# ethereum/pos-evolution

Hardware: AMD Instinct MI355X
Metric: attestations aggregated/sec + get_head() p50 latency at 1M validators (higher is better)
Workload: dtype int32

## Files before the change

pos_evolution_amd/csrc/engine_g1.cpp:

```cpp
#include "engine_internal.h"

using namespace posevo;

namespace posevo {

void g1_stream_guard(pe_engine* h, hipStream_t s)
{
    if (h->side_ever && s != h->side_stream && s != h->fin_stream && s != h->norm_stream) (void)hipStreamWaitEvent(s, h->ev_join, 0);
}

int build_points30(pe_engine* h, uint64_t n)
{
    HIP_TRY(h, h->d_points30.ensure(std::max<size_t>(128, 4ull * G1_ROW_WORDS * n)));
    launch_g1_table_s30(h->stream, h->d_points.as<uint32_t>(), h->d_points30.as<uint32_t>(), n);
    HIP_TRY(h, hipGetLastError());
    h->points30_valid = true;
    return PE_OK;
}

int launch_g1_planned(pe_engine* h, const uint32_t* d_points, const uint32_t* d_members, const uint32_t* d_bits,
                      const G1Group* d_groups, const G1Plan& plan, uint8_t* d_out96, uint32_t* dev_jac,
                      hipStream_t s, hipStream_t fin, DevBuf* partials, DevBuf* lane_partials, const AttPlan* plan_dev,
                      const uint32_t* d_members1, uint64_t caller_rows, const G1Complement* cm)
{
    if (plan.n_groups == 0) return PE_OK;
    if (!s) s = h->stream;
    if (!fin) fin = s;
    if (!partials) partials = &h->d_partials;
    if (!lane_partials) lane_partials = &h->d_lane_partials;
    PE_TRY(ensure_quiesced(h, *partials,
                           std::max<size_t>(PE_G1_PARTIAL_BYTES, (size_t)PE_G1_PARTIAL_BYTES * plan.n_partials)));
    const size_t lane_bytes = (size_t)G1_LANE_PARTIAL_BYTES * G1_WG * ((plan.n_slots + G1_WG - 1) / G1_WG);
    PE_TRY(ensure_quiesced(h, *lane_partials, std::max<size_t>(PE_G1_PARTIAL_BYTES, lane_bytes)));
    const uint32_t* d_points30;
    if (d_points == h->d_points.as<uint32_t>()) {
        if (!h->points30_valid) return fail(h, PE_ERR_STATE, "the registry's table of the accumulation's field form was not built");
        d_points30 = h->d_points30.as<uint32_t>();
    } else {
        const uint64_t n_rows = caller_rows;
        if (d_points != h->d_tmp_points.as<uint32_t>() || 4ull * G1_ROW_WORDS * n_rows > h->d_tmp_points.cap)
            return fail(h, PE_ERR_STATE, "G1 sum over an unknown point table");
        HIP_TRY(h, h->d_tmp_points30.ensure(std::max<size_t>(128, 4ull * G1_ROW_WORDS * n_rows)));
        launch_g1_table_s30(s, d_points, h->d_tmp_points30.as<uint32_t>(), n_rows);
        d_points30 = h->d_tmp_points30.as<uint32_t>();
    }
    const bool chain = fin != s && fin == h->fin_stream;
    const int exclusive = chain && h->tune.exclusive && h->blocks.size() <= 4096 ? 1 : 0;
    {
        const bool skip = !h->prof_timeline && s != h->stream && (h->acc_launches++ & 3) != 0;
        ProfScope ps(h, PE_KERNEL_G1_ACCUMULATE, s, skip);
        unsigned long long* clock_rec = nullptr;
        if (h->profiling) {
            if (!h->acc_clock && hipHostMalloc(reinterpret_cast<void**>(&h->acc_clock), 16ull * pe_engine::ACC_CLOCK_RING,
                                               hipHostMallocDefault) != hipSuccess) {
                (void)hipGetLastError();
                h->acc_clock = nullptr;
            }
            if (h->acc_clock) {
                clock_rec = h->acc_clock + 2 * (h->acc_clock_n++ % pe_engine::ACC_CLOCK_RING);
                clock_rec[0] = clock_rec[1] = 0;
            }
        }
        launch_g1_accumulate(s, d_points30, d_members, d_bits, d_groups, plan.n_groups, plan.n_slots,
                             lane_partials->as<uint32_t>(), partials->as<uint32_t>(), plan_dev, d_members1, exclusive, clock_rec,
                             cm ? cm->cmpl : nullptr);
    }
    hipStream_t ts = fin;
    if (ts != s) {
        HIP_TRY(h, hipEventRecord(h->ev_acc, s));
        HIP_TRY(h, hipStreamWaitEvent(ts, h->ev_acc, 0));
    }
    {
        ProfScope ps(h, PE_KERNEL_G1_TREE, ts);
        launch_g1_tree(ts, lane_partials->as<uint32_t>(), d_groups, plan.n_groups, plan.n_slots, partials->as<uint32_t>(),
                       ts != s ? 1 : 0,
                       plan_dev, exclusive);
    }
    hipStream_t ns = fin;
    if (chain && h->norm_stream) {
        ns = h->norm_stream;
        HIP_TRY(h, hipEventRecord(h->ev_tree, ts));
        HIP_TRY(h, hipStreamWaitEvent(ns, h->ev_tree, 0));
    } else if (ts != fin) {
        HIP_TRY(h, hipEventRecord(h->ev_tree, ts));
        HIP_TRY(h, hipStreamWaitEvent(fin, h->ev_tree, 0));
    }
    if (cm)
        for (int t = 0; t < 2; ++t)
            if (cm->ev[t]) HIP_TRY(h, hipStreamWaitEvent(ns, cm->ev[t], 0));
    {
        ProfScope ps(h, PE_KERNEL_G1_NORMALISE, ns);
        launch_g1_finish(ns, partials->as<uint32_t>(), d_groups, plan.n_groups, 0, 0, d_out96, dev_jac, plan_dev,
                         cm ? cm->cmpl : nullptr, cm ? cm->sums[0] : nullptr, cm ? cm->sums[1] : nullptr);
    }
    HIP_TRY(h, hipGetLastError());
    return PE_OK;
}

void committee_sums_drop(pe_engine* h)
{
    for (auto& t : h->tables) t.sums_valid = t.sums_wanted = false;
    if (h->sums_stream) (void)hipStreamSynchronize(h->sums_stream);
}
int build_committee_sums(pe_engine* h, CommitteeTable* t, bool defer)
{
    t->sums_valid = false;
    t->sums_wanted = false;
    if (!h->tune.committee_sums || !t->is_partition || !h->have_points || !h->points30_valid || h->dist_ready()) return PE_OK;
    if (t->n_committees == 0 || t->n_val_at_load != h->n_val || t->offsets.size() != (size_t)t->n_committees + 1) return PE_OK;
// ... 681 lines not shown
```

pos_evolution_amd/csrc/engine_internal.h:

```cpp
#pragma once
#include <hip/hip_runtime.h>
#include <dlfcn.h>
#include <rccl/rccl.h>

#include <algorithm>
#include <array>
#include <chrono>
#include <cstdlib>
#include <map>
#include <cstdio>
#include <cstddef>
#include <cstring>
#include <functional>
#include <memory>
#include <new>
#include <numeric>
#include <string>
#include <thread>
#include <unordered_map>
#include <vector>

#include "../../include/posevo.h"
#include "../../include/posevo_profile.h"
#include "att_row.h"
// ... 330 lines not shown
    };
    std::vector<SigSeg> sig_batch;
    hipEvent_t ev_sig = nullptr;
    hipEvent_t ev_fork = nullptr, ev_join = nullptr;
    bool side_busy = false;
    bool side_ever = false;
    bool streaming = false;
    std::vector<std::function<int()>> deferred;
    struct HeldFc {
        bool active = false;
        int arena = -1;
        bool have_fc = false;
        bool have_head = false;
        ValidateFcArgs validate{};
        LmdVmArgs lmd{};
        VotesArgs votes{};
        TreeArgs tree{};
        std::function<int()> between;
        std::vector<std::function<int()>> g1;
        bool fence_pending = false;
    } held;
    bool pairing = std::getenv("POSEVO_PAIR") == nullptr || std::atoi(std::getenv("POSEVO_PAIR")) != 0;
    struct Tune {
        static int env(const char* name, int dflt)
        {
            const char* e = std::getenv(name);
            return e && *e ? std::atoi(e) : dflt;
        }
        int exclusive = env("POSEVO_ACC_EXCLUSIVE", 1);
        int state_on = env("POSEVO_STATE_ON", 2);
        int sig_batch = env("POSEVO_SIG_BATCH", 8);
        int queue_probe = env("POSEVO_QUEUE_PROBE", 1);
        int committee_sums = env("POSEVO_COMMITTEE_SUMS", 1);
        uint32_t ssz_tile_log2 = (uint32_t)std::min<int>(SSZ_TILE_LOG2, std::max<int>(SSZ_TILE_LOG2_MIN, env("POSEVO_SSZ_TILE_LOG2", SSZ_TILE_LOG2)));
    } tune;

    struct ResGroup { uint32_t byte_off, n_bits, word, sig_valid, tag; };
    std::vector<ResGroup> res_groups;
    std::shared_ptr<std::vector<uint32_t>> res_info_host;
    bool res_valid = false;
    int res_arena = 0;
    uint64_t res_generation = 0;

    struct ResidentRows {
        bool valid = false;
        int arena = 0;
        uint32_t n_in = 0;
        const void* rows = nullptr;
        TablesDev tables{};
        uint64_t generation = 0;
        int set = 0;
        uint32_t n_groups = 0;
    } rr;

    int g1_tune_calls = 0;
    float g1_tune_best[2] = {1e30f, 1e30f};
    uint32_t g1_target_slots = 0;
    hipEvent_t g1_tune_ev[2] = {nullptr, nullptr};
    bool points30_valid = false;
    DevBuf d_points30, d_tmp_points30;

    ncclComm_t comm = nullptr, comm_g1 = nullptr;
    int early_rc = PE_OK;
    uint32_t xchg_blocks = 0;
    uint64_t xchg_nval = 0;
    bool last_agg_on_side = false;
// ... 300 lines not shown
            d.slot_base = cursor;
            d.out_base = outp;
            continue;
        }
        if (d.n_tasks <= wg_slots) {
            uint32_t l2 = 0;
            while ((1u << l2) < d.n_tasks) ++l2;
            d.log2_block = l2;
            const uint32_t blk = 1u << l2;
            cursor = (cursor + blk - 1) & ~(blk - 1);
            d.slot_base = cursor;
            cursor += blk;
            d.out_base = outp;
            outp += 1;
        } else {
            d.log2_block = 9;
            cursor = (cursor + wg_slots - 1) & ~(wg_slots - 1);
            d.slot_base = cursor;
            const uint32_t wgs = (d.n_tasks + wg_slots - 1) / wg_slots;
            cursor += wgs * wg_slots;
            d.out_base = outp;
            outp += wgs;
        }
    }
    plan->n_groups = n_groups;
    plan->n_slots = cursor;
    plan->n_partials = outp;
}

void g1_stream_guard(pe_engine* h, hipStream_t s);
int build_points30(pe_engine* h, uint64_t n);
struct G1Complement {
    const uint32_t* cmpl = nullptr;
    const uint32_t* sums[2] = {nullptr, nullptr};
    hipEvent_t ev[2] = {nullptr, nullptr};
};
int launch_g1_planned(pe_engine* h, const uint32_t* d_points, const uint32_t* d_members, const uint32_t* d_bits,
                      const G1Group* d_groups, const G1Plan& plan, uint8_t* d_out96, uint32_t* dev_jac,
                      hipStream_t s = nullptr, hipStream_t fin = nullptr, DevBuf* partials = nullptr,
                      DevBuf* lane_partials = nullptr, const AttPlan* plan_dev = nullptr,
                      const uint32_t* d_members1 = nullptr, uint64_t caller_rows = 0, const G1Complement* cm = nullptr);
int build_committee_sums(pe_engine* h, CommitteeTable* t, bool defer);
int committee_sums_build_wanted(pe_engine* h, CommitteeTable* t);
void committee_sums_drop(pe_engine* h);

struct Resolved {
    CommitteeTable* table = nullptr;
    uint32_t pos = 0;
    uint32_t size = 0;
    uint32_t block_idx = 0;
};
inline CommitteePos resolve_committee(const pe_engine* h, CommitteeTable* t, const pe_attestation& a, Resolved* out)
{
    const CommitteePos cp = att_committee_pos(t->n_committees, h->cfg.slots_per_epoch, a.slot, a.index);
    if (cp.exists) {
        out->table = t;
        out->pos = cp.pos;
        out->size = t->offsets[cp.pos + 1] - t->offsets[cp.pos];
    }
    return cp;
}

struct BatchMemo {
    struct Slot { uint8_t root[32]; uint32_t idx; uint32_t used; };
    Slot slots[256];
    std::vector<uint64_t> anc;
// ... 91 lines not shown
```

pos_evolution_amd/csrc/engine_resident.cpp:

```cpp
#include "engine_internal.h"


using namespace posevo;

namespace posevo {

namespace {

struct RrLayout {
    AttPlan* plan;
    uint32_t *slot_of, *rep_of, *gid_of_row, *ubytes, *member_row;
    PlanSync* sync;
    PlanRec* rec;
    AttGroup* grp;
    UnionGroup* ug;
    G1Group* g1;
    AttRow *rows_fc, *rows_st;
    int32_t *status_fc, *status_st;
    uint32_t* cmpl;
    uint32_t *crow_start[2], *crow_cursor[2], *crow_cnt[2], *crow_list[2];
    size_t bytes;
};

RrLayout rr_layout(uint8_t* base, uint32_t cap_n, uint32_t cap_c)
// ... 181 lines not shown
    const uint32_t slot_cap = std::max<uint32_t>(2 * G1_TARGET_LANES, (n + G1_WG - 1) / G1_WG * G1_WG);
    const size_t words_cap = (size_t)out_arena_cap / 4 + n + 16;
    Stage st(h);
    PE_TRY(st.reserve((size_t)arena_len + 256));
    const size_t pad_at = ((size_t)arena_len + 15) & ~size_t(15);
    const size_t off_arena = st.alloc(pad_at + 32);
    if (set == 0) {
        PE_TRY(ensure_quiesced_arenas(h, &pe_engine::PipeArena::d_res_bits, words_cap * 4 + 64));
        PE_TRY(ensure_quiesced_arenas(h, &pe_engine::PipeArena::d_res_info, 8ull * n + 64));
    } else {
        PE_TRY(ensure_quiesced(h, RS.bits, words_cap * 4 + 64));
        PE_TRY(ensure_quiesced(h, RS.info, 8ull * n + 64));
    }
    OutBlock ob(h);
    const size_t off_plan = ob.alloc(sizeof(AttPlan));
    const size_t off_rows = ob.alloc(sizeof(pe_attestation) * (size_t)n);
    const size_t off_gof = ob.alloc(4ull * n);
    const size_t off_obits = ob.alloc(words_cap * 4);
    const size_t off_oinfo = ob.alloc(8ull * n);
    const size_t off_opk = out_aggpk96 ? ob.alloc(96ull * n) : 0;
    G1Complement cm;
    bool by_cmpl = false;
    if (out_aggpk96 && !dev_partials && set == 0 && h->tune.committee_sums && !h->dist_ready())
        for (int t = 0; t < 2; ++t) {
            if (tabs[t]) PE_TRY(committee_sums_build_wanted(h, tabs[t]));
            if (tabs[t] && tabs[t]->sums_valid && tabs[t]->d_sums.p && tabs[t]->ev_sums) {
                cm.sums[t] = tabs[t]->d_sums.as<uint32_t>();
                cm.ev[t] = tabs[t]->ev_sums;
                by_cmpl = true;
            }
        }
    const size_t off_ocm = by_cmpl ? ob.alloc(4ull * n) : 0;
    PE_TRY(ob.ensure());
    if (by_cmpl) cm.cmpl = L.cmpl;
    if (want_pk) {
        PE_TRY(ensure_quiesced_arenas(h, &pe_engine::PipeArena::d_partials, std::max<size_t>(PE_G1_PARTIAL_BYTES, (size_t)PE_G1_PARTIAL_BYTES * n)));
        PE_TRY(ensure_quiesced_arenas(h, &pe_engine::PipeArena::d_lane_partials, (size_t)G1_LANE_PARTIAL_BYTES * slot_cap));
        PE_TRY(ensure_quiesced(h, h->d_partials, std::max<size_t>(PE_G1_PARTIAL_BYTES, (size_t)PE_G1_PARTIAL_BYTES * n)));
        PE_TRY(ensure_quiesced(h, h->d_lane_partials, (size_t)G1_LANE_PARTIAL_BYTES * slot_cap));
    }
    lap.mark("ragg.1_reserve");
    *out_n_groups = 0;
    AttPlan* plan_host = ob.host<AttPlan>(off_plan);
    memset(plan_host, 0, sizeof(AttPlan));
    plan_host->error = 0xFFFFFFFFu;
    const MemKind arena_kind = arena_len ? mem_kind(bits_arena) : MemKind::Pageable;
    hipStream_t ms = h->stream;
    const bool pair_ok = h->held.active && h->held.arena != h->cur && set == 0 && !n_dev && hold_eligible(h);
    if (h->held.active && !pair_ok) PE_TRY(held_issue(h));
    if (set == 0) {
        if (!h->deferred.empty()) PE_TRY(run_deferred(h));
        if (A.side_used) HIP_TRY(h, hipStreamWaitEvent(ms, h->ev_join, 0));
        if (sig_batch_holds(h, h->cur)) PE_TRY(sig_batch_flush(h));
        if (A.leg_used) HIP_TRY(h, hipStreamWaitEvent(ms, A.ev_leg, 0));
        PE_TRY(aux_join(h, ms));
    }
    h->res_valid = false;
    h->rr.valid = false;
    const size_t deferred_before = h->deferred.size();
    struct Unwind {
        pe_engine* h; size_t keep; bool armed = true;
        ~Unwind() { if (armed) { h->rr.valid = false; if (h->deferred.size() > keep) h->deferred.resize(keep); } }
    } unwind{h, deferred_before};
    bool ingest_copies = false;
    if (arena_kind == MemKind::Pageable) {
        memcpy(st.host<uint8_t>(off_arena), bits_arena, arena_len);
        memset(st.host<uint8_t>(off_arena) + arena_len, 0, pad_at + 32 - arena_len);
// ... 328 lines not shown
```

pos_evolution_amd/csrc/g1_kernels.hip:

```cpp
#define POSEVO_FP_MUL_CALLED 1
#include <algorithm>
#include <hip/hip_ext.h>
#include "g1.h"
#include "g1_s30.h"
#include "fp_sqrt.h"
#include "kernels.h"

namespace posevo {

__global__ void __launch_bounds__(256) k_g1_convert(const uint8_t* __restrict__ be96, uint32_t* __restrict__ mont24,
                                                     uint64_t n)
{
    uint64_t i = (uint64_t)blockIdx.x * blockDim.x + threadIdx.x;
    if (i >= n) return;
    const uint8_t* src = be96 + 96 * i;
    uint32_t* dst = mont24 + (uint64_t)G1_ROW_WORDS * i;
    if (src[0] & 0x40) {
#pragma unroll
        for (int j = 0; j < 24; ++j) dst[j] = 0;
        return;
    }
    fp x, y, xm, ym;
    fp_load_be48(x, src);
    fp_load_be48(y, src + 48);
    y.l[11] = __builtin_bswap32(reinterpret_cast<const uint32_t*>(src + 48)[0]);
    fp_to_mont(xm, x);
    fp_to_mont(ym, y);
#pragma unroll
    for (int j = 0; j < 12; ++j) {
        dst[j] = xm.l[j];
        dst[12 + j] = ym.l[j];
    }
}

void launch_g1_convert(hipStream_t s, const uint8_t* be96, uint32_t* mont24, uint64_t n)
{
    if (n == 0) return;
    hipLaunchKernelGGL(k_g1_convert, dim3((unsigned)((n + 255) / 256)), dim3(256), 0, s, be96, mont24, n);
}
// ... 162 lines not shown
__device__ __forceinline__ void global_store_x(uint32_t* __restrict__ dst, const g1x& p)
{
    global_store_fp(dst, p.x);
    global_store_fp(dst + 12, p.y);
    global_store_fp(dst + 24, p.zz);
    global_store_fp(dst + 36, p.zzz);
}
__device__ __forceinline__ void global_load_x(g1x& p, const uint32_t* __restrict__ src)
{
    global_load_fp(p.x, src);
    global_load_fp(p.y, src + 12);
    global_load_fp(p.zz, src + 24);
    global_load_fp(p.zzz, src + 36);
}

__device__ __forceinline__ uint32_t find_group(const G1Group* __restrict__ groups, uint32_t n_groups, uint32_t slot)
{
    uint32_t lo = 0, hi = n_groups;
    {
        const uint32_t lb = groups[0].log2_block;
        const uint32_t g0 = min(lb <= 8 ? slot >> lb : 0u, n_groups - 1);
        if (groups[g0].slot_base <= slot) {
            if (g0 + 1 == n_groups || groups[g0 + 1].slot_base > slot) return g0;
            lo = g0 + 1;
        } else {
            hi = g0;
        }
    }
    while (hi - lo > 1) {
        uint32_t mid = (lo + hi) >> 1;
        if (groups[mid].slot_base <= slot) lo = mid; else hi = mid;
    }
    return lo;
}

#ifdef POSEVO_G1_PHASE_TIMING
__device__ unsigned long long g1_phase_stamps[16 * 4096];
#define G1_STAMP(i) do { if (threadIdx.x == 0 && blockIdx.x < 4096) g1_phase_stamps[blockIdx.x * 16 + (i)] = wall_clock64(); } while (0)
__device__ unsigned long long g1_wave_info[3 * 4 * 4096];
#define G1_WAVE_BEGIN() do { if ((threadIdx.x & 63) == 0 && blockIdx.x < 4096) { \
        unsigned long long* w_ = &g1_wave_info[3 * (blockIdx.x * 4 + (threadIdx.x >> 6))]; \
        w_[0] = (unsigned long long)__builtin_amdgcn_s_getreg((4) | (0 << 6) | (31 << 11)) | \
                ((unsigned long long)__builtin_amdgcn_s_getreg((20) | (0 << 6) | (31 << 11)) << 32); \
        w_[1] = wall_clock64(); } } while (0)
#define G1_WAVE_END() do { if ((threadIdx.x & 63) == 0 && blockIdx.x < 4096) \
        g1_wave_info[3 * (blockIdx.x * 4 + (threadIdx.x >> 6)) + 2] = wall_clock64(); } while (0)
#else
#define G1_WAVE_BEGIN() do { } while (0)
#define G1_WAVE_END() do { } while (0)
#define G1_STAMP(i) do { } while (0)
#endif

namespace s30 {
__device__ __noinline__ fq fq_mul_nc(int32_t a0, int32_t a1, int32_t a2, int32_t a3, int32_t a4, int32_t a5, int32_t a6,
                                     int32_t a7, int32_t a8, int32_t a9, int32_t a10, int32_t a11, int32_t a12,
                                     int32_t b0, int32_t b1, int32_t b2, int32_t b3, int32_t b4, int32_t b5, int32_t b6,
                                     int32_t b7, int32_t b8, int32_t b9, int32_t b10, int32_t b11, int32_t b12)
{
    const fq a = {{a0, a1, a2, a3, a4, a5, a6, a7, a8, a9, a10, a11, a12}};
    const fq b = {{b0, b1, b2, b3, b4, b5, b6, b7, b8, b9, b10, b11, b12}};
    fq r;
    fq_mul(r, a, b);
    return r;
}
__device__ __noinline__ fq fq_sqr_nc(int32_t a0, int32_t a1, int32_t a2, int32_t a3, int32_t a4, int32_t a5, int32_t a6,
                                     int32_t a7, int32_t a8, int32_t a9, int32_t a10, int32_t a11, int32_t a12)
// ... 146 lines not shown
    fq_from_lane(t2, m4, base);
    fq_sub_norm(tmp, m4, t2);
    fq_select(sel, q == 1, m3, m4);
    fq_select(out_a, q == 2, X3, sel);
    out_b = tmp;
    return true;
}

__device__ __forceinline__ void g1_slot_block(const G1Group* __restrict__ groups, uint32_t n_groups, uint32_t n_slots,
                                              uint32_t slot, uint32_t& my_out, uint32_t& my_size, G1Group& d, uint32_t& t,
                                              uint32_t* g_out = nullptr)
{
    my_out = NONE32;
    my_size = 0;
    t = 0;
    if (slot >= n_slots) return;
    const uint32_t g = find_group(groups, n_groups, slot);
    if (g_out) *g_out = g;
    d = groups[g];
    t = slot - d.slot_base;
    const bool wide = d.log2_block > 8;
    const uint32_t block_slots = d.n_tasks == 0 ? 0u
                               : wide ? ((d.n_tasks + G1_WG - 1) / G1_WG) * G1_WG : (1u << d.log2_block);
    if (t < block_slots) {
        my_size = wide ? (uint32_t)G1_WG : (1u << d.log2_block);
        my_out = d.out_base + (wide ? (t >> 8) : 0u);
    }
}


template <bool SOLO>
__device__ __forceinline__ void g1_tree_body(const uint32_t* __restrict__ lane_partials, const G1Group* __restrict__ groups,
                                             uint32_t n_groups, uint32_t n_slots, uint32_t* __restrict__ wg_partials,
                                             const AttPlan* __restrict__ plan_dev)
{
    if (SOLO) asm volatile("" ::: "a7");
    if (plan_dev) {
        n_groups = plan_dev->n_groups;
        n_slots = plan_dev->n_slots;
    }
    extern __shared__ __attribute__((aligned(16))) uint32_t lds[];
    uint32_t* lds_out = lds + G1S_WORDS * G1_WG;
    uint32_t* lds_sz = lds_out + G1_WG;
    const int tid = threadIdx.x;
    for (uint32_t wg = blockIdx.x; wg * G1_WG < n_slots; wg += gridDim.x) {
    const uint32_t slot = wg * G1_WG + tid;
    uint32_t my_out, my_size, t;
    G1Group d{};
    g1_slot_block(groups, n_groups, n_slots, slot, my_out, my_size, d, t);
    if (my_size == 1) my_size = 0;
    {
        const uint32_t* b = lane_partials + (size_t)wg * G1S_WORDS * G1_WG + tid;
#pragma unroll
        for (int k = 0; k < G1S_WORDS; ++k) lds[k * G1_WG + tid] = b[k * G1_WG];
    }
    lds_out[tid] = my_out;
    lds_sz[tid] = my_size;
    __syncthreads();
    G1_STAMP(2);
#ifdef POSEVO_G1_PHASE_TIMING
    int g1_level = 0;
#endif
    for (int n = G1_WG / 2; n >= 1; n >>= 1) {
        if (n <= G1_WG / 4) {
            const int w = tid >> 2, q = tid & 3;
            const bool active = w < n;
            fq out_a, out_b;
            uint32_t out = NONE32, sz = 0;
            bool store_lds = false;
            if (active) {
                sz = lds_sz[2 * w];
                out = lds_out[2 * w];
                if (sz >= 2) {
                    fq a, b;
                    lds_load_fq(a, lds, q >> 1, 2 * w + (q & 1));
                    lds_load_fq(b, lds, 2 + (q >> 1), 2 * w + ((q & 1) ^ 1));
                    const unsigned long long inf_lanes = __ballot(fq_limbs_zero(b));
                    bool fast = ((inf_lanes >> ((tid & 63) & ~3)) & 0xFull) == 0;
                    if (fast) fast = g1s_add_quad(out_a, out_b, q, a, b);
                    if (!fast) {
                        g1q p1, p2;
                        lds_load_q(p1, lds, 2 * w);
                        lds_load_q(p2, lds, 2 * w + 1);
                        g1q_add_full(p1, p2);
                        if (p1.inf) g1q_set_inf(p1);
                        fq sel;
                        fq_select(sel, q == 1, p1.zz, p1.zzz);
                        fq_select(out_a, q == 2, p1.x, sel);
                        out_b = p1.y;
                    }
                    sz >>= 1;
// ... 67 lines not shown
                    global_store_fq_as_mont32(dst, out_a);
                    global_store_fq_as_mont32(dst + 12, out_b);
                    sz = 0;
                } else {
                    store_lds = true;
                }
            } else {
                sz = 0;
            }
        }
        __syncthreads();
        if (active) {
            if (store_lds) {
                lds_store_fq(lds, role ? 2 : 0, w, out_a);
                lds_store_fq(lds, role ? 3 : 1, w, out_b);
            }
            if (!role) {
                lds_out[w] = out;
                lds_sz[w] = sz;
            }
        }
        __syncthreads();
#ifdef POSEVO_G1_PHASE_TIMING
        G1_STAMP(3 + g1_level);
        ++g1_level;
#endif
    }
    }
}
}

__global__ void __launch_bounds__(G1_WG) __attribute__((amdgpu_waves_per_eu(2, 2)))
k_g1_tree(const uint32_t* __restrict__ lane_partials, const G1Group* __restrict__ groups, uint32_t n_groups,
          uint32_t n_slots, uint32_t* __restrict__ wg_partials, const AttPlan* __restrict__ plan_dev)
{
    s30::g1_tree_body<false>(lane_partials, groups, n_groups, n_slots, wg_partials, plan_dev);
}
__global__ void __launch_bounds__(G1_WG) __attribute__((amdgpu_waves_per_eu(1, 1), amdgpu_num_vgpr(256)))
k_g1_tree_solo(const uint32_t* __restrict__ lane_partials, const G1Group* __restrict__ groups, uint32_t n_groups,
               uint32_t n_slots, uint32_t* __restrict__ wg_partials, const AttPlan* __restrict__ plan_dev)
{
    s30::g1_tree_body<true>(lane_partials, groups, n_groups, n_slots, wg_partials, plan_dev);
}

__global__ void __launch_bounds__(256)
k_g1_table_s30(const uint32_t* __restrict__ pts32, uint32_t* __restrict__ pts30, uint64_t n)
{
    using s30::FQ_N;
    const uint64_t i = (uint64_t)blockIdx.x * 256 + threadIdx.x;
    if (i >= n) return;
    const uint32_t* src = pts32 + (uint64_t)G1_ROW_WORDS * i;
    uint32_t w[24], any = 0;
#pragma unroll
    for (int k = 0; k < 24; ++k) { w[k] = src[k]; any |= w[k]; }
    uint32_t* dst = pts30 + (uint64_t)G1_ROW_WORDS * i;
    s30::fq x, y;
    s30::fq_set_zero(x);
    s30::fq_set_zero(y);
    if (any) {
        s30::fq_from_mont32(x, w);
        s30::fq_from_mont32(y, w + 12);
    }
#pragma unroll
    for (int k = 0; k < FQ_N; ++k) { dst[k] = (uint32_t)x.l[k]; dst[FQ_N + k] = (uint32_t)y.l[k]; }
    dst[2 * FQ_N] = any ? 1u : 0u;
#pragma unroll
    for (int k = 2 * FQ_N + 1; k < G1_ROW_WORDS; ++k) dst[k] = 0;
}

namespace s30 {
static_assert(2 * FQ_N + 1 <= 28, "a row of the S30 table is read as seven 16-byte vectors");
__device__ __forceinline__ bool load_point_s30(fq& x, fq& y, const uint32_t* __restrict__ pts30, uint32_t idx)
{
    const uint4* p = reinterpret_cast<const uint4*>(pts30 + (uint64_t)G1_ROW_WORDS * idx);
    const uint4 v0 = p[0], v1 = p[1], v2 = p[2], v3 = p[3], v4 = p[4], v5 = p[5], v6 = p[6];
    x.l[0] = v0.x; x.l[1] = v0.y; x.l[2] = v0.z; x.l[3] = v0.w;
    x.l[4] = v1.x; x.l[5] = v1.y; x.l[6] = v1.z; x.l[7] = v1.w;
    x.l[8] = v2.x; x.l[9] = v2.y; x.l[10] = v2.z; x.l[11] = v2.w;
    x.l[12] = v3.x;
    y.l[0] = v3.y; y.l[1] = v3.z; y.l[2] = v3.w;
    y.l[3] = v4.x; y.l[4] = v4.y; y.l[5] = v4.z; y.l[6] = v4.w;
    y.l[7] = v5.x; y.l[8] = v5.y; y.l[9] = v5.z; y.l[10] = v5.w;
    y.l[11] = v6.x; y.l[12] = v6.y;
    return v6.z != 0;
}
}

namespace s30 {
__device__ __forceinline__ void g1_accumulate_body(const uint32_t* __restrict__ pts30, const uint32_t* __restrict__ members,
                                                   const uint32_t* __restrict__ bit_arena, const G1Group* __restrict__ groups,
                                                   uint32_t n_groups, uint32_t n_slots, uint32_t* __restrict__ lane_partials,
                                                   uint32_t* __restrict__ wg_partials, const AttPlan* __restrict__ plan_dev,
                                                   const uint32_t* __restrict__ members1,
                                                   unsigned long long* __restrict__ clock_rec,
                                                   const uint32_t* __restrict__ cmpl)
{
    const int tid = threadIdx.x;
    if (plan_dev) {
        n_groups = plan_dev->n_groups;
        n_slots = plan_dev->n_slots;
        if (blockIdx.x * G1_WG >= n_slots) return;
    }
    unsigned long long rec_w0 = 0, rec_c0 = 0;
    if (clock_rec && blockIdx.x == 0) {
        rec_w0 = wall_clock64();
        rec_c0 = clock64();
    }
    const uint32_t slot = blockIdx.x * G1_WG + tid;
    G1_STAMP(0);
    G1_WAVE_BEGIN();
#ifdef POSEVO_ACC_PRIO_LEVEL
    __builtin_amdgcn_s_setprio(POSEVO_ACC_PRIO_LEVEL);
#endif
    g1q acc;
    g1q_set_inf(acc);
    bool exc = false;
    uint32_t my_out, my_size, t;
    G1Group d{};
    uint32_t g = 0;
    g1_slot_block(groups, n_groups, n_slots, slot, my_out, my_size, d, t, &g);
    uint32_t first = 0, count = 0;
    uint32_t invert = 0;
    if (slot < n_slots && t < d.n_tasks) {
        const uint32_t gk = d.k & 0x7FFFFFFFu;
        if (d.k >> 31) members = members1;
        first = t * gk;
        count = min(gk, d.n_members - first);
        if (cmpl) invert = cmpl[g] != NONE32 ? 1u : 0u;
    }
    const bool gated = d.bits_word != NONE32;
    auto want = [&](uint32_t j, uint32_t& idx) -> bool {
        const uint32_t i = first + j;
        idx = members ? members[d.member_start + i] : d.member_start + i;
        if (!gated) return true;
        return (((bit_arena[d.bits_word + (i >> 5)] >> (i & 31)) & 1u) ^ invert) != 0;
    };
    auto fetch = [&](uint32_t j, fq& ox, fq& oy) -> bool {
        uint32_t idx;
        if (!want(j, idx)) return false;
        return load_point_s30(ox, oy, pts30, idx);
    };
    {
        fq qx, qy, nx, ny;
        bool have = false, nhave = false, w1 = false, w2 = false;
        uint32_t i1 = 0, i2 = 0;
        if (count > 0) {
            uint32_t i0;
            if (want(0, i0)) have = load_point_s30(qx, qy, pts30, i0);
        }
        if (count > 1) w1 = want(1, i1);
        for (uint32_t j = 0; j < count; ++j) {
            w2 = false;
            if (j + 2 < count) w2 = want(j + 2, i2);
            nhave = false;
            if (w1) nhave = load_point_s30(nx, ny, pts30, i1);
            if (have) {
                if (acc.inf) g1q_set_first(acc, qx, qy);
                else g1q_madd_fast(acc, qx, qy, exc);
            }
            qx = nx; qy = ny; have = nhave;
            i1 = i2; w1 = w2;
// ... 12 lines not shown
    const bool inf = acc.inf;
#pragma unroll
    for (int k = 0; k < FQ_N; ++k) {
        b[k * G1_WG] = inf ? 0u : (uint32_t)acc.x.l[k];
        b[(FQ_N + k) * G1_WG] = inf ? 0u : (uint32_t)acc.y.l[k];
        b[(2 * FQ_N + k) * G1_WG] = inf ? 0u : (uint32_t)acc.zz.l[k];
        b[(3 * FQ_N + k) * G1_WG] = inf ? 0u : (uint32_t)acc.zzz.l[k];
    }
    if (my_size == 1) {
        uint32_t* dst = wg_partials + (size_t)G1X_WORDS * my_out;
#pragma nounroll
        for (int c = 0; c < 4; ++c) {
            uint32_t w[12];
            fq_to_mont32_via<FqCalled>(w, acc.x);
#pragma unroll
            for (int k = 0; k < 12; ++k) dst[12 * c + k] = inf ? 0u : w[k];
            acc.x = acc.y;
            acc.y = acc.zz;
            acc.zz = acc.zzz;
        }
    }
    if (clock_rec && blockIdx.x == 0 && tid == 0) {
        clock_rec[0] = wall_clock64() - rec_w0;
        clock_rec[1] = clock64() - rec_c0;
    }
}
}

__global__ void __launch_bounds__(G1_WG) __attribute__((amdgpu_waves_per_eu(2, 2)))
k_g1_accumulate(const uint32_t* __restrict__ pts30, const uint32_t* __restrict__ members,
                const uint32_t* __restrict__ bit_arena, const G1Group* __restrict__ groups, uint32_t n_groups,
                uint32_t n_slots, uint32_t* __restrict__ lane_partials, uint32_t* __restrict__ wg_partials,
                const AttPlan* __restrict__ plan_dev, const uint32_t* __restrict__ members1,
                unsigned long long* __restrict__ clock_rec, const uint32_t* __restrict__ cmpl)
{
    s30::g1_accumulate_body(pts30, members, bit_arena, groups, n_groups, n_slots, lane_partials, wg_partials, plan_dev,
                            members1, clock_rec, cmpl);
}

void launch_g1_table_s30(hipStream_t s, const uint32_t* points_mont24, uint32_t* points_s30, uint64_t n)
{
    if (n == 0) return;
    hipLaunchKernelGGL(k_g1_table_s30, dim3((unsigned)((n + 255) / 256)), dim3(256), 0, s, points_mont24, points_s30, n);
}
void launch_g1_accumulate(hipStream_t s, const uint32_t* points_s30, const uint32_t* members,
                              const uint32_t* bit_arena, const G1Group* groups, uint32_t n_groups, uint32_t n_slots,
                              uint32_t* lane_partials, uint32_t* wg_partials48, const AttPlan* plan_dev,
                              const uint32_t* members1, int exclusive, unsigned long long* clock_rec, const uint32_t* cmpl)
{
    if (n_groups == 0 || n_slots == 0) return;
    const unsigned blocks = (n_slots + G1_WG - 1) / G1_WG;
    size_t lds_bytes = 0;
    if (exclusive) {
        lds_bytes = G1_ACC_EXCLUSIVE_LDS;
        if (first_use_on_this_device<82>())
            (void)hipFuncSetAttribute(reinterpret_cast<const void*>(k_g1_accumulate), hipFuncAttributeMaxDynamicSharedMemorySize,
                                      (int)G1_ACC_EXCLUSIVE_LDS);
    }
    hipLaunchKernelGGL(k_g1_accumulate, dim3(blocks), dim3(G1_WG), lds_bytes, s, points_s30, members, bit_arena,
                       groups, n_groups, n_slots, lane_partials, wg_partials48, plan_dev, members1, clock_rec, cmpl);
}

void launch_g1_tree(hipStream_t s, const uint32_t* lane_partials, const G1Group* groups, uint32_t n_groups,
                    uint32_t n_slots, uint32_t* wg_partials48, int one_per_cu, const AttPlan* plan_dev, int solo)
{
    if (n_groups == 0 || n_slots == 0) return;
    const unsigned blocks = (n_slots + G1_WG - 1) / G1_WG;
    size_t lds_bytes = (s30::G1S_WORDS + 2) * G1_WG * sizeof(uint32_t);
    if (solo) {
        hipLaunchKernelGGL(k_g1_tree_solo, dim3(blocks), dim3(G1_WG), lds_bytes, s, lane_partials, groups, n_groups, n_slots,
                           wg_partials48, plan_dev);
        return;
    }
    if (one_per_cu) {
        constexpr size_t padded = 84 * 1024;
        if (first_use_on_this_device<84>())
            (void)hipFuncSetAttribute(reinterpret_cast<const void*>(k_g1_tree), hipFuncAttributeMaxDynamicSharedMemorySize,
                                      (int)padded);
        lds_bytes = padded;
    }
    hipLaunchKernelGGL(k_g1_tree, dim3(blocks), dim3(G1_WG), lds_bytes, s, lane_partials, groups, n_groups, n_slots,
                       wg_partials48, plan_dev);
}

__global__ void __launch_bounds__(64)
k_g1_finish(const uint32_t* __restrict__ partials, const G1Group* __restrict__ groups, uint32_t n_groups,
            uint32_t n_parts_fixed, uint32_t part_stride, uint8_t* __restrict__ out_be96,
            uint32_t* __restrict__ out_jac, const AttPlan* __restrict__ plan_dev, const uint32_t* __restrict__ cmpl,
            const uint32_t* __restrict__ sums0, const uint32_t* __restrict__ sums1)
{
    if (plan_dev) n_groups = min(n_groups, plan_dev->n_groups);
    const uint32_t g = blockIdx.x * blockDim.x + threadIdx.x;
    if (g >= n_groups) return;
    uint32_t first, n_parts, stride;
    if (groups) {
        const G1Group d = groups[g];
        first = d.out_base;
        n_parts = d.log2_block > 8 ? (d.n_tasks + G1_WG - 1) / G1_WG : 1u;
        if (d.n_tasks == 0) n_parts = 0;
        stride = 1;
    } else {
        first = g;
        n_parts = n_parts_fixed;
        stride = part_stride;
    }
    const uint32_t verdict = cmpl ? cmpl[g] : NONE32;
    const uint32_t* csum = nullptr;
    if (verdict != NONE32) csum = ((verdict >> 31) ? sums1 : sums0) + (size_t)G1X_WORDS * (verdict & 0x7FFFFFFFu);
    g1x acc;
    g1x_set_inf(acc);
    for (uint32_t k = 0; k < n_parts + (csum ? 1u : 0u); ++k) {
        g1x q;
        const uint32_t* src = partials + (size_t)G1X_WORDS * (first + (uint64_t)k * stride);
        if (k == n_parts) {
            fp ny;
// ... 59 lines not shown
```

pos_evolution_amd/csrc/kernels.h:

```cpp
#pragma once
#include <hip/hip_runtime.h>
#include <stdint.h>

namespace posevo {

template <int TAG>
static bool first_use_on_this_device()
{
    static bool done[64] = {false};
    int dev = 0;
    (void)hipGetDevice(&dev);
    if (dev < 0 || dev >= 64) return true;
    if (done[dev]) return false;
    done[dev] = true;
    return true;
}

constexpr uint32_t NONE32 = 0xFFFFFFFFu;
constexpr int G1_ROW_WORDS = 32;
constexpr int G2_WG_SLOTS = 128;
constexpr int G1_WG = 256;
constexpr int G1_LANE_PARTIAL_BYTES = 208;
constexpr int TREE_MAX_BLOCKS = 8192;
constexpr int VOTES_MAX_WG = 256;

struct G1Group {
    uint32_t member_start;
    uint32_t n_members;
    uint32_t bits_word;
    uint32_t slot_base;
    uint32_t n_tasks;
    uint32_t k;
    uint32_t log2_block;
    uint32_t out_base;
};

void launch_g1_convert(hipStream_t s, const uint8_t* be96, uint32_t* mont24, uint64_t n);
void launch_g1_table_s30(hipStream_t s, const uint32_t* points_mont24, uint32_t* points_s30, uint64_t n);
struct AttPlan;
void launch_g1_accumulate(hipStream_t s, const uint32_t* points_s30, const uint32_t* members,
                          const uint32_t* bit_arena, const G1Group* groups, uint32_t n_groups, uint32_t n_slots,
                          uint32_t* lane_partials, uint32_t* wg_partials48, const AttPlan* plan_dev = nullptr,
                          const uint32_t* members1 = nullptr, int exclusive = 0, unsigned long long* clock_rec = nullptr,
                          const uint32_t* cmpl = nullptr);
void launch_g1_committee_groups(hipStream_t s, const uint32_t* offsets, uint32_t n_committees, uint32_t k, uint32_t log2_block,
                                G1Group* groups);
constexpr size_t G1_ACC_EXCLUSIVE_LDS = 82 * 1024;
void launch_g1_tree(hipStream_t s, const uint32_t* lane_partials, const G1Group* groups, uint32_t n_groups,
                    uint32_t n_slots, uint32_t* wg_partials48, int one_per_cu = 0, const AttPlan* plan_dev = nullptr,
                    int solo = 0);
void launch_g1_finish(hipStream_t s, const uint32_t* partials48, const G1Group* groups, uint32_t n_groups,
                      uint32_t n_parts_fixed, uint32_t part_stride, uint8_t* out_be96, uint32_t* out_xyzz48,
                      const AttPlan* plan_dev = nullptr, const uint32_t* cmpl = nullptr, const uint32_t* sums0 = nullptr,
                      const uint32_t* sums1 = nullptr);

struct TreeDev {
    const uint32_t* size;
    const uint32_t* parent;
    const uint32_t* rank;
    const uint8_t* leaf_ok;
    const uint32_t* pos_of_idx;
    const uint32_t* idx_of_pos;
    uint32_t n;
};
struct VoteTotals {
    unsigned long long total_active_balance;
    unsigned long long num_active;
};

struct AttRow {
    uint32_t member_base;
    uint32_t n_bits;
    uint32_t bits_word;
    uint32_t block_idx;
    uint32_t epoch_p1;
    uint32_t order;
    uint32_t flag_mask;
    uint32_t which;
    uint32_t slot;
    uint32_t gate;
};
void launch_lmd_update(hipStream_t s, const AttRow* rows, uint32_t n_rows, const uint32_t* members,
                       const uint32_t* bit_arena, const uint8_t* flags, uint64_t* vote_key, uint32_t* vote_block,
// ... 431 lines not shown
```

Before: 5.542 billion.

## Add sparse-absentee path summing only missing members for near-full committees

For committees aggregated by complement where few members are absent, a new one-wave-per-group kernel scans the bitfield, lists the absent indices, sums only those points, and writes the group's partial directly. The main accumulate and tree kernels then skip those groups, and the tree uses a barrier-or to exit early when a workgroup has nothing to reduce. This is meant to avoid full per-member accumulation when participation is high. The cost is an extra kernel launch and a dependence on the correctness of the complement-sum path.

```diff
diff --git a/pos_evolution_amd/csrc/engine_g1.cpp b/pos_evolution_amd/csrc/engine_g1.cpp
--- a/pos_evolution_amd/csrc/engine_g1.cpp
+++ b/pos_evolution_amd/csrc/engine_g1.cpp
@@ -46,6 +46,11 @@
     }
     const bool chain = fin != s && fin == h->fin_stream;
     const int exclusive = chain && h->tune.exclusive && h->blocks.size() <= 4096 ? 1 : 0;
+    const uint32_t sparse_max = cm && cm->info ? h->tune.g1_sparse_max() : 0u;
+    const uint32_t* sparse_info = sparse_max ? cm->info : nullptr;
+    if (sparse_max)
+        launch_g1_absentees(s, d_points30, d_members, d_members1, d_bits, d_groups, plan.n_groups, plan_dev, cm->cmpl, sparse_info,
+                            sparse_max, partials->as<uint32_t>());
     {
         const bool skip = !h->prof_timeline && s != h->stream && (h->acc_launches++ & 3) != 0;
         ProfScope ps(h, PE_KERNEL_G1_ACCUMULATE, s, skip);
@@ -63,7 +68,7 @@
         }
         launch_g1_accumulate(s, d_points30, d_members, d_bits, d_groups, plan.n_groups, plan.n_slots,
                              lane_partials->as<uint32_t>(), partials->as<uint32_t>(), plan_dev, d_members1, exclusive, clock_rec,
-                             cm ? cm->cmpl : nullptr);
+                             cm ? cm->cmpl : nullptr, sparse_info, sparse_max);
     }
     hipStream_t ts = fin;
     if (ts != s) {
@@ -74,7 +79,7 @@
         ProfScope ps(h, PE_KERNEL_G1_TREE, ts);
         launch_g1_tree(ts, lane_partials->as<uint32_t>(), d_groups, plan.n_groups, plan.n_slots, partials->as<uint32_t>(),
                        ts != s ? 1 : 0,
-                       plan_dev, exclusive);
+                       plan_dev, exclusive, sparse_max ? cm->cmpl : nullptr, sparse_info, sparse_max);
     }
     hipStream_t ns = fin;
     if (chain && h->norm_stream) {
diff --git a/pos_evolution_amd/csrc/engine_internal.h b/pos_evolution_amd/csrc/engine_internal.h
--- a/pos_evolution_amd/csrc/engine_internal.h
+++ b/pos_evolution_amd/csrc/engine_internal.h
@@ -386,6 +386,11 @@
         int sig_batch = env("POSEVO_SIG_BATCH", 8);
         int queue_probe = env("POSEVO_QUEUE_PROBE", 1);
         int committee_sums = env("POSEVO_COMMITTEE_SUMS", 1);
+        int g1_sparse = env("POSEVO_G1_SPARSE", 1);
+        uint32_t g1_sparse_max() const
+        {
+            return g1_sparse <= 0 ? 0u : g1_sparse == 1 ? G1_SPARSE_MAX : std::min<uint32_t>((uint32_t)g1_sparse, G1_SPARSE_CAP);
+        }
         uint32_t ssz_tile_log2 = (uint32_t)std::min<int>(SSZ_TILE_LOG2, std::max<int>(SSZ_TILE_LOG2_MIN, env("POSEVO_SSZ_TILE_LOG2", SSZ_TILE_LOG2)));
     } tune;
 
@@ -752,6 +757,7 @@
 int build_points30(pe_engine* h, uint64_t n);
 struct G1Complement {
     const uint32_t* cmpl = nullptr;
+    const uint32_t* info = nullptr;
     const uint32_t* sums[2] = {nullptr, nullptr};
     hipEvent_t ev[2] = {nullptr, nullptr};
 };
diff --git a/pos_evolution_amd/csrc/engine_resident.cpp b/pos_evolution_amd/csrc/engine_resident.cpp
--- a/pos_evolution_amd/csrc/engine_resident.cpp
+++ b/pos_evolution_amd/csrc/engine_resident.cpp
@@ -237,7 +237,10 @@
         }
     const size_t off_ocm = by_cmpl ? ob.alloc(4ull * n) : 0;
     PE_TRY(ob.ensure());
-    if (by_cmpl) cm.cmpl = L.cmpl;
+    if (by_cmpl) {
+        cm.cmpl = L.cmpl;
+        cm.info = RS.info.as<uint32_t>();
+    }
     if (want_pk) {
         PE_TRY(ensure_quiesced_arenas(h, &pe_engine::PipeArena::d_partials, std::max<size_t>(PE_G1_PARTIAL_BYTES, (size_t)PE_G1_PARTIAL_BYTES * n)));
         PE_TRY(ensure_quiesced_arenas(h, &pe_engine::PipeArena::d_lane_partials, (size_t)G1_LANE_PARTIAL_BYTES * slot_cap));
diff --git a/pos_evolution_amd/csrc/g1_kernels.hip b/pos_evolution_amd/csrc/g1_kernels.hip
--- a/pos_evolution_amd/csrc/g1_kernels.hip
+++ b/pos_evolution_amd/csrc/g1_kernels.hip
@@ -5,6 +5,7 @@
 #include "g1_s30.h"
 #include "fp_sqrt.h"
 #include "kernels.h"
+#include "wave64.h"
 
 namespace posevo {
 
@@ -233,6 +234,15 @@
         if (groups[mid].slot_base <= slot) lo = mid; else hi = mid;
     }
     return lo;
+}
+
+__device__ __forceinline__ bool g1_group_sparse(const G1Group& d, uint32_t g, const uint32_t* __restrict__ cmpl,
+                                                const uint32_t* __restrict__ info, uint32_t sparse_max)
+{
+    if (!cmpl || !info || sparse_max == 0) return false;
+    if (cmpl[g] == NONE32 || d.log2_block > 8 || d.bits_word == NONE32) return false;
+    const uint32_t present = info[2 * g];
+    return present <= d.n_members && d.n_members - present <= min(sparse_max, G1_SPARSE_CAP);
 }
 
 #ifdef POSEVO_G1_PHASE_TIMING
@@ -445,7 +455,8 @@
 template <bool SOLO>
 __device__ __forceinline__ void g1_tree_body(const uint32_t* __restrict__ lane_partials, const G1Group* __restrict__ groups,
                                              uint32_t n_groups, uint32_t n_slots, uint32_t* __restrict__ wg_partials,
-                                             const AttPlan* __restrict__ plan_dev)
+                                             const AttPlan* __restrict__ plan_dev, const uint32_t* __restrict__ cmpl,
+                                             const uint32_t* __restrict__ sparse_info, uint32_t sparse_max)
 {
     if (SOLO) asm volatile("" ::: "a7");
     if (plan_dev) {
@@ -460,8 +471,10 @@
     const uint32_t slot = wg * G1_WG + tid;
     uint32_t my_out, my_size, t;
     G1Group d{};
-    g1_slot_block(groups, n_groups, n_slots, slot, my_out, my_size, d, t);
+    uint32_t g = 0;
+    g1_slot_block(groups, n_groups, n_slots, slot, my_out, my_size, d, t, &g);
     if (my_size == 1) my_size = 0;
+    if (my_size && g1_group_sparse(d, g, cmpl, sparse_info, sparse_max)) my_size = 0;
     {
         const uint32_t* b = lane_partials + (size_t)wg * G1S_WORDS * G1_WG + tid;
 #pragma unroll
@@ -469,7 +482,7 @@
     }
     lds_out[tid] = my_out;
     lds_sz[tid] = my_size;
-    __syncthreads();
+    if (!__syncthreads_or(my_size != 0)) continue;
     G1_STAMP(2);
 #ifdef POSEVO_G1_PHASE_TIMING
     int g1_level = 0;
@@ -603,15 +616,17 @@
 
 __global__ void __launch_bounds__(G1_WG) __attribute__((amdgpu_waves_per_eu(2, 2)))
 k_g1_tree(const uint32_t* __restrict__ lane_partials, const G1Group* __restrict__ groups, uint32_t n_groups,
-          uint32_t n_slots, uint32_t* __restrict__ wg_partials, const AttPlan* __restrict__ plan_dev)
-{
-    s30::g1_tree_body<false>(lane_partials, groups, n_groups, n_slots, wg_partials, plan_dev);
+          uint32_t n_slots, uint32_t* __restrict__ wg_partials, const AttPlan* __restrict__ plan_dev,
+          const uint32_t* __restrict__ cmpl, const uint32_t* __restrict__ sparse_info, uint32_t sparse_max)
+{
+    s30::g1_tree_body<false>(lane_partials, groups, n_groups, n_slots, wg_partials, plan_dev, cmpl, sparse_info, sparse_max);
 }
 __global__ void __launch_bounds__(G1_WG) __attribute__((amdgpu_waves_per_eu(1, 1), amdgpu_num_vgpr(256)))
 k_g1_tree_solo(const uint32_t* __restrict__ lane_partials, const G1Group* __restrict__ groups, uint32_t n_groups,
-               uint32_t n_slots, uint32_t* __restrict__ wg_partials, const AttPlan* __restrict__ plan_dev)
-{
-    s30::g1_tree_body<true>(lane_partials, groups, n_groups, n_slots, wg_partials, plan_dev);
+               uint32_t n_slots, uint32_t* __restrict__ wg_partials, const AttPlan* __restrict__ plan_dev,
+               const uint32_t* __restrict__ cmpl, const uint32_t* __restrict__ sparse_info, uint32_t sparse_max)
+{
+    s30::g1_tree_body<true>(lane_partials, groups, n_groups, n_slots, wg_partials, plan_dev, cmpl, sparse_info, sparse_max);
 }
 
 __global__ void __launch_bounds__(256)
@@ -664,7 +679,8 @@
                                                    uint32_t* __restrict__ wg_partials, const AttPlan* __restrict__ plan_dev,
                                                    const uint32_t* __restrict__ members1,
                                                    unsigned long long* __restrict__ clock_rec,
-                                                   const uint32_t* __restrict__ cmpl)
+                                                   const uint32_t* __restrict__ cmpl,
+                                                   const uint32_t* __restrict__ sparse_info, uint32_t sparse_max)
 {
     const int tid = threadIdx.x;
     if (plan_dev) {
@@ -698,6 +714,10 @@
         first = t * gk;
         count = min(gk, d.n_members - first);
         if (cmpl) invert = cmpl[g] != NONE32 ? 1u : 0u;
+        if (invert && g1_group_sparse(d, g, cmpl, sparse_info, sparse_max)) {
+            count = 0;
+            my_size = 0;
+        }
     }
     const bool gated = d.bits_word != NONE32;
     auto want = [&](uint32_t j, uint32_t& idx) -> bool {
@@ -776,10 +796,11 @@
                 const uint32_t* __restrict__ bit_arena, const G1Group* __restrict__ groups, uint32_t n_groups,
                 uint32_t n_slots, uint32_t* __restrict__ lane_partials, uint32_t* __restrict__ wg_partials,
                 const AttPlan* __restrict__ plan_dev, const uint32_t* __restrict__ members1,
-                unsigned long long* __restrict__ clock_rec, const uint32_t* __restrict__ cmpl)
+                unsigned long long* __restrict__ clock_rec, const uint32_t* __restrict__ cmpl,
+                const uint32_t* __restrict__ sparse_info, uint32_t sparse_max)
 {
     s30::g1_accumulate_body(pts30, members, bit_arena, groups, n_groups, n_slots, lane_partials, wg_partials, plan_dev,
-                            members1, clock_rec, cmpl);
+                            members1, clock_rec, cmpl, sparse_info, sparse_max);
 }
 
 void launch_g1_table_s30(hipStream_t s, const uint32_t* points_mont24, uint32_t* points_s30, uint64_t n)
@@ -790,7 +811,8 @@
 void launch_g1_accumulate(hipStream_t s, const uint32_t* points_s30, const uint32_t* members,
                               const uint32_t* bit_arena, const G1Group* groups, uint32_t n_groups, uint32_t n_slots,
                               uint32_t* lane_partials, uint32_t* wg_partials48, const AttPlan* plan_dev,
-                              const uint32_t* members1, int exclusive, unsigned long long* clock_rec, const uint32_t* cmpl)
+                              const uint32_t* members1, int exclusive, unsigned long long* clock_rec, const uint32_t* cmpl,
+                              const uint32_t* sparse_info, uint32_t sparse_max)
 {
     if (n_groups == 0 || n_slots == 0) return;
     const unsigned blocks = (n_slots + G1_WG - 1) / G1_WG;
@@ -802,18 +824,20 @@
                                       (int)G1_ACC_EXCLUSIVE_LDS);
     }
     hipLaunchKernelGGL(k_g1_accumulate, dim3(blocks), dim3(G1_WG), lds_bytes, s, points_s30, members, bit_arena,
-                       groups, n_groups, n_slots, lane_partials, wg_partials48, plan_dev, members1, clock_rec, cmpl);
+                       groups, n_groups, n_slots, lane_partials, wg_partials48, plan_dev, members1, clock_rec, cmpl, sparse_info,
+                       sparse_max);
 }
 
 void launch_g1_tree(hipStream_t s, const uint32_t* lane_partials, const G1Group* groups, uint32_t n_groups,
-                    uint32_t n_slots, uint32_t* wg_partials48, int one_per_cu, const AttPlan* plan_dev, int solo)
+                    uint32_t n_slots, uint32_t* wg_partials48, int one_per_cu, const AttPlan* plan_dev, int solo,
+                    const uint32_t* cmpl, const uint32_t* sparse_info, uint32_t sparse_max)
 {
     if (n_groups == 0 || n_slots == 0) return;
     const unsigned blocks = (n_slots + G1_WG - 1) / G1_WG;
     size_t lds_bytes = (s30::G1S_WORDS + 2) * G1_WG * sizeof(uint32_t);
     if (solo) {
         hipLaunchKernelGGL(k_g1_tree_solo, dim3(blocks), dim3(G1_WG), lds_bytes, s, lane_partials, groups, n_groups, n_slots,
-                           wg_partials48, plan_dev);
+                           wg_partials48, plan_dev, cmpl, sparse_info, sparse_max);
         return;
     }
     if (one_per_cu) {
@@ -824,7 +848,111 @@
         lds_bytes = padded;
     }
     hipLaunchKernelGGL(k_g1_tree, dim3(blocks), dim3(G1_WG), lds_bytes, s, lane_partials, groups, n_groups, n_slots,
-                       wg_partials48, plan_dev);
+                       wg_partials48, plan_dev, cmpl, sparse_info, sparse_max);
+}
+
+namespace s30 {
+__device__ __forceinline__ void g1q_from_lane_down(g1q& q, const g1q& p, int off)
+{
+#pragma unroll
+    for (int j = 0; j < FQ_N; ++j) {
+        q.x.l[j] = __shfl_down(p.x.l[j], off, 64);
+        q.y.l[j] = __shfl_down(p.y.l[j], off, 64);
+        q.zz.l[j] = __shfl_down(p.zz.l[j], off, 64);
+        q.zzz.l[j] = __shfl_down(p.zzz.l[j], off, 64);
+    }
+    q.inf = __shfl_down((int)p.inf, off, 64) != 0;
+    q.affine = false;
+}
+__device__ __forceinline__ void g1_absentees_body(const uint32_t* __restrict__ pts30, const uint32_t* __restrict__ members,
+                                                  const uint32_t* __restrict__ members1,
+                                                  const uint32_t* __restrict__ bit_arena, const G1Group* __restrict__ groups,
+                                                  uint32_t n_groups, const AttPlan* __restrict__ plan_dev,
+                                                  const uint32_t* __restrict__ cmpl,
+                                                  const uint32_t* __restrict__ sparse_info, uint32_t sparse_max,
+                                                  uint32_t* __restrict__ wg_partials)
+{
+    __shared__ uint32_t list[G1_SPARSE_CAP];
+    if (plan_dev) n_groups = min(n_groups, plan_dev->n_groups);
+    const uint32_t g = blockIdx.x;
+    if (g >= n_groups) return;
+    const G1Group d = groups[g];
+    if (!g1_group_sparse(d, g, cmpl, sparse_info, sparse_max)) return;
+    const uint32_t lane = threadIdx.x;
+    const uint32_t n_words = (d.n_members + 31) >> 5;
+    const uint32_t tail_mask = (d.n_members & 31) ? ((1u << (d.n_members & 31)) - 1u) : 0xFFFFFFFFu;
+    uint32_t total = 0;
+    for (uint32_t w0 = 0; w0 < n_words; w0 += 64) {
+        const uint32_t w = w0 + lane;
+        uint32_t absent = 0;
+        if (w < n_words) absent = ~bit_arena[d.bits_word + w] & (w == n_words - 1 ? tail_mask : 0xFFFFFFFFu);
+        const uint32_t mine = (uint32_t)__builtin_popcount(absent);
+        uint32_t pos = total + wave_incl_scan(mine) - mine;
+        while (absent) {
+            if (pos < G1_SPARSE_CAP) list[pos] = 32u * w + (uint32_t)__builtin_ctz(absent);
+            ++pos;
+            absent &= absent - 1;
+        }
+        total += wave_sum(mine);
+    }
+    total = min(total, G1_SPARSE_CAP);
+    __syncthreads();
+    const uint32_t* __restrict__ mem = (d.k >> 31) ? members1 : members;
+    g1q acc;
+    g1q_set_inf(acc);
+    for (uint32_t e = lane; e < total; e += 64) {
+        const uint32_t i = list[e];
+        const uint32_t idx = mem ? mem[d.member_start + i] : d.member_start + i;
+        fq qx, qy;
+        const bool have = load_point_s30(qx, qy, pts30, idx);
+        g1q_add_affine<FqCalled>(acc, qx, qy, !have);
+    }
+    uint32_t live = min(total, 64u);
+#pragma nounroll
+    for (uint32_t off = 32; off >= 1; off >>= 1) {
+        if (live <= off) continue;
+        g1q q;
+        g1q_from_lane_down(q, acc, (int)off);
+        if (lane < off && lane + off < live) g1q_add<FqCalled>(acc, q);
+        live = off;
+    }
+    fq coord;
+#pragma unroll
+    for (int j = 0; j < FQ_N; ++j) {
+        const int32_t x = __shfl(acc.x.l[j], 0, 64), y = __shfl(acc.y.l[j], 0, 64);
+        const int32_t zz = __shfl(acc.zz.l[j], 0, 64), zzz = __shfl(acc.zzz.l[j], 0, 64);
+        coord.l[j] = lane == 0 ? x : lane == 1 ? y : lane == 2 ? zz : zzz;
+    }
+    const bool inf = __shfl((int)acc.inf, 0, 64) != 0;
+    if (lane < 4) {
+        uint32_t w[12];
+        fq_to_mont32_via<FqCalled>(w, coord);
+        uint4* dst = reinterpret_cast<uint4*>(wg_partials + (size_t)G1X_WORDS * d.out_base + 12 * lane);
+        dst[0] = inf ? make_uint4(0, 0, 0, 0) : make_uint4(w[0], w[1], w[2], w[3]);
+        dst[1] = inf ? make_uint4(0, 0, 0, 0) : make_uint4(w[4], w[5], w[6], w[7]);
+        dst[2] = inf ? make_uint4(0, 0, 0, 0) : make_uint4(w[8], w[9], w[10], w[11]);
+    }
+}
+}
+
+__global__ void __launch_bounds__(64) __attribute__((amdgpu_waves_per_eu(2, 8)))
+k_g1_absentees(const uint32_t* __restrict__ pts30, const uint32_t* __restrict__ members,
+               const uint32_t* __restrict__ members1, const uint32_t* __restrict__ bit_arena,
+               const G1Group* __restrict__ groups, uint32_t n_groups, const AttPlan* __restrict__ plan_dev,
+               const uint32_t* __restrict__ cmpl, const uint32_t* __restrict__ sparse_info, uint32_t sparse_max,
+               uint32_t* __restrict__ wg_partials)
+{
+    s30::g1_absentees_body(pts30, members, members1, bit_arena, groups, n_groups, plan_dev, cmpl, sparse_info, sparse_max,
+                           wg_partials);
+}
+
+void launch_g1_absentees(hipStream_t s, const uint32_t* points_s30, const uint32_t* members, const uint32_t* members1,
+                         const uint32_t* bit_arena, const G1Group* groups, uint32_t n_groups, const AttPlan* plan_dev,
+                         const uint32_t* cmpl, const uint32_t* sparse_info, uint32_t sparse_max, uint32_t* wg_partials48)
+{
+    if (n_groups == 0 || !cmpl || !sparse_info || sparse_max == 0) return;
+    hipLaunchKernelGGL(k_g1_absentees, dim3(n_groups), dim3(64), 0, s, points_s30, members, members1, bit_arena, groups,
+                       n_groups, plan_dev, cmpl, sparse_info, sparse_max, wg_partials48);
 }
 
 __global__ void __launch_bounds__(64)
diff --git a/pos_evolution_amd/csrc/kernels.h b/pos_evolution_amd/csrc/kernels.h
--- a/pos_evolution_amd/csrc/kernels.h
+++ b/pos_evolution_amd/csrc/kernels.h
@@ -42,13 +42,19 @@
                           const uint32_t* bit_arena, const G1Group* groups, uint32_t n_groups, uint32_t n_slots,
                           uint32_t* lane_partials, uint32_t* wg_partials48, const AttPlan* plan_dev = nullptr,
                           const uint32_t* members1 = nullptr, int exclusive = 0, unsigned long long* clock_rec = nullptr,
-                          const uint32_t* cmpl = nullptr);
+                          const uint32_t* cmpl = nullptr, const uint32_t* sparse_info = nullptr, uint32_t sparse_max = 0);
 void launch_g1_committee_groups(hipStream_t s, const uint32_t* offsets, uint32_t n_committees, uint32_t k, uint32_t log2_block,
                                 G1Group* groups);
+constexpr uint32_t G1_SPARSE_MAX = 128;
+constexpr uint32_t G1_SPARSE_CAP = 256;
+void launch_g1_absentees(hipStream_t s, const uint32_t* points_s30, const uint32_t* members, const uint32_t* members1,
+                         const uint32_t* bit_arena, const G1Group* groups, uint32_t n_groups, const AttPlan* plan_dev,
+                         const uint32_t* cmpl, const uint32_t* sparse_info, uint32_t sparse_max, uint32_t* wg_partials48);
 constexpr size_t G1_ACC_EXCLUSIVE_LDS = 82 * 1024;
 void launch_g1_tree(hipStream_t s, const uint32_t* lane_partials, const G1Group* groups, uint32_t n_groups,
                     uint32_t n_slots, uint32_t* wg_partials48, int one_per_cu = 0, const AttPlan* plan_dev = nullptr,
-                    int solo = 0);
+                    int solo = 0, const uint32_t* cmpl = nullptr, const uint32_t* sparse_info = nullptr,
+                    uint32_t sparse_max = 0);
 void launch_g1_finish(hipStream_t s, const uint32_t* partials48, const G1Group* groups, uint32_t n_groups,
                       uint32_t n_parts_fixed, uint32_t part_stride, uint8_t* out_be96, uint32_t* out_xyzz48,
                       const AttPlan* plan_dev = nullptr, const uint32_t* cmpl = nullptr, const uint32_t* sums0 = nullptr,
```

Result: faster. 6.737 billion, median of 6 (+21.6%).
